# mbari-org/ecoz2rs

Hardware: AMD Instinct MI355X
Metric: vq_learn_frames_per_sec_M1024_P36 (higher is better)
Workload: dtype f64

## Files before the change

### ecoz2rs_amd/csrc/vq_pass.cpp

```cpp
#include "vq_session.h"


int e2vq_pass_mode(const e2vq_session* s)
{
    if (e2vq::uses_mfma(s->NC) && !e2vq::mfma_is_wide(s->NC)) {
        const long images = 8L * 16 * (2 * s->NC + 5 + 3) * 4;
        if ((long)s->M * s->RS * 8 + images + 2048 <= E2VQ_LDS_BYTES && s->M <= 128) return 1;
        if (s->M <= 4 * e2vq::mfma_hybrid_cells(s->NC)) return 5;
        return 2;
    }
    return 2;
}

int e2vq_fold_pending_timing(e2vq_session* s)
{
    if (!s->timing_pending) return 0;
    float ms = 0.f;
    HIPCHK(hipEventElapsedTime(&ms, s->ev0, s->ev1));
    s->timing_sum_ms += ms;
    s->timing_count += 1;
    if (s->timing_mid) HIPCHK(hipEventElapsedTime(&ms, s->ev0, s->ev_mid));
    s->timing_sweep_ms += ms;
    s->timing_mid = false;
    s->timing_pending = false;
// ... 300 lines not shown
{
    if (kind) *kind = s->last_prefiltered ? s->last_kind : 0;
    if (two_stage) *two_stage = s->last_two_stage ? 1 : 0;
    if (flagged_fraction) *flagged_fraction = s->last_flagged_frac;
    return 0;
}

extern "C" int e2vq_sweep_executed(e2vq_session* s, int64_t* flagged, int64_t* jobs, int64_t* one_stage_jobs, int reset)
{
    HIPCHK(hipSetDevice(s->device));
    u64 dev[2] = {0, 0};
    if (s->d_sort) {
        HIPCHK(hipMemcpyAsync(dev, e2vq::sweep_totals_of(s->d_sort), sizeof dev, hipMemcpyDeviceToHost, s->stream));
        if (reset) HIPCHK(hipMemsetAsync(e2vq::sweep_totals_of(s->d_sort), 0, sizeof dev, s->stream));
        HIPCHK(hipStreamSynchronize(s->stream));
    }
    if (flagged) *flagged = (int64_t)(dev[0] + s->sw_host_flagged);
    if (jobs) *jobs = (int64_t)(dev[1] + s->sw_host_jobs);
    if (one_stage_jobs) *one_stage_jobs = (int64_t)s->sw_one_stage_jobs;
    if (reset) s->sw_host_flagged = s->sw_host_jobs = s->sw_one_stage_jobs = 0;
    return 0;
}

extern "C" int e2vq_set_sweep_policy(e2vq_session* s, double two_stage_max_fraction, double max_uncertified_fraction)
{
    if (two_stage_max_fraction >= 0.0) s->two_stage_max_frac = two_stage_max_fraction;
    if (max_uncertified_fraction >= 0.0) s->pre_max_uncertified = max_uncertified_fraction;
    s->two_stage_off_until_M = 0;
    s->pre_off_from_M = 0;
    return 0;
}

extern "C" int e2vq_sweep_policy_state(e2vq_session* s, int* one_stage_until_M, int* plain_from_M, int64_t* uncertified)
{
    if (one_stage_until_M) *one_stage_until_M = s->two_stage_off_until_M;
    if (plain_from_M) *plain_from_M = s->pre_off_from_M;
    if (uncertified) *uncertified = s->last_fb;
    return 0;
}

extern "C" int e2vq_last_pass_info(e2vq_session* s, int* prefiltered, int64_t* fallback_frames)
{
    HIPCHK(hipSetDevice(s->device));
    if (prefiltered) *prefiltered = s->last_prefiltered ? 1 : 0;
    if (fallback_frames) {
        int n = 0;
// ... 222 lines not shown
        s->lstats_dirty = true;
        e2vq::launch_codebook_prepare(s->d_refl_spec, s->M, s->NC, s->d_cbq_spec, s->d_l1max_spec, s->d_cbm_spec,
                                      s->stream);
    }
    HIPCHK(hipGetLastError());
    s->spec_valid = true;
    if (spin_for_sequence(s, &s->h_stats->seq, "statistics kernel", &s->stats_wait_s)) return 1;
    if (s->rec_pending) {
        s->rec_last_total = s->h_stats->rec_total;
        s->rec_pending = false;
    }
    if (fused) {
        s->last_fb = s->last_prefiltered ? (i64)s->h_stats->fb : -1;
        const double limit = s->last_first_of_level ? std::min(1.0, 1.5 * s->pre_max_uncertified) : s->pre_max_uncertified;
        if (s->last_fb >= 0 && s->T > 0 && (double)s->last_fb > limit * (double)s->T &&
            (!s->pre_off_from_M || s->M < s->pre_off_from_M))
            s->pre_off_from_M = s->M;
    }
    if (s->sw_pending) {
        const u64 fl = s->h_stats->sw_flagged, jobs = s->h_stats->sw_jobs;
        s->sw_pending = false;
        s->sw_host_flagged += fl;
        s->sw_host_jobs += jobs;
        s->last_flagged_frac = jobs ? (double)fl / (double)jobs : -1.0;
        if (jobs && s->last_flagged_frac > s->two_stage_max_frac) s->two_stage_off_until_M = s->M;
        if (jobs && s->last_flagged_frac > 0.8 && s->last_flagged_frac > s->two_stage_max_frac)
            s->two_stage_off_until_M = (s->last_flagged_frac > 0.98 ? 4 : 2) * s->M;
    }
    i64 l[8] = {0, 0, 0, 0, 0, 0, 0, 0};
    for (int slot = 0; slot < 64; ++slot)
        for (int k = 0; k < 8; ++k) l[k] += s->h_stats->l[slot * 8 + k];
    double l1max;
    memcpy(&l1max, &s->h_stats->l1bits, 8);
    const int Ed = e2vq::dist_exponent(s->h_sc.maxabs, l1max);
    const double DD = e2vq::unfix(l[0], l[1], 30 - Ed);
    const double SS = e2vq::unfix(l[2], l[3], 30 - 2 * Ed);
    const double T = (double)s->T_total;
    const double avg = DD / T;
    const double q = SS / T;
    const double p = avg * avg;
    double v = q - p;
    if (!(v > 0.0)) v = 0.0;
    double w = 0.0;
    for (int m = 0; m < s->M; ++m) w += s->h_within[m];
    s->last.M = s->M;
    s->last.DD = DD;
// ... 62 lines not shown
```

### ecoz2rs_amd/csrc/vq_session.h

```cpp
#pragma once
#include "../../include/ecoz2_vq.h"
#include "hip_host.h"
#include "vq_device.h"
#include "vq_fixed.h"
#include "vq_io.h"
#include <hip/hip_runtime.h>
#include <dlfcn.h>
#include <errno.h>
#include <float.h>
#include <math.h>
#include <stdarg.h>
#include <stdint.h>
#include <stdio.h>
#include <stdlib.h>
#include <string.h>
#include <algorithm>
#include <chrono>
#include <atomic>
#include <condition_variable>
#include <memory>
#include <mutex>
#include <shared_mutex>
#include <string>
#include <thread>
// ... 6 lines not shown

struct e2vq_session {
    int device = 0, P = 0, NC = 0, FB = 64, RS = 0, NPAD = 0;
    hipStream_t own_stream = nullptr, stream = nullptr;
    double* d_blk = nullptr;
    double* d_aos = nullptr;
    i64 T = 0, nblocks = 0, T_total = 0;
    bool prepared = false;
    bool maxabs_scanned = false;
    int M = 0, M_cap = 0;
    double* d_refl = nullptr;
    double* d_refl_next = nullptr;
    double* d_cbq = nullptr;
    double* d_cbm = nullptr;
    double* d_cbT = nullptr;
    u64* d_l1max = nullptr;
    double* d_refl_spec = nullptr;
    double* d_cbq_spec = nullptr;
    double* d_cbm_spec = nullptr;
    u64* d_l1max_spec = nullptr;
    bool spec_valid = false;
    bool spec_zeroed = false;
    hipEvent_t ev_stats = nullptr;
    struct HostStats { i64 l[64 * 8]; u64 l1bits; volatile u64 seq; i64 failed; volatile u64 seq2; volatile u64 err; volatile i64 rec_total; volatile u64 sw_flagged, sw_jobs; volatile i64 fb; }* h_stats = nullptr;
    long verified_passes = 0;
    bool verify_publish = false;
    bool failed_pending = false;
    e2vq_level_stats* failed_patch = nullptr;
    u64 stats_seq = 0;
    double stats_wait_s = 0.0;
    double* h_within = nullptr;
    DevScalars* d_sc = nullptr;
    DevScalars h_sc{};
    u64* d_maxabs = nullptr;
    int* d_flags = nullptr;
    i64* d_stats = nullptr;
    i64* d_rows = nullptr;
    double* d_S = nullptr;
    double* d_within = nullptr;
    i64* d_lstats = nullptr;
    bool lstats_dirty = false;
    bool stats_valid = false;
    bool rows_fresh = false;
    e2vq_level_stats last{};
    double DDprv = DBL_MAX / 1e5;
    double* d_qaos = nullptr;
    double* d_qblk = nullptr;
// ... 41 lines not shown
    bool rec_enabled = true;
    int rec_min_M = 64;
    size_t rec_max_bytes = (size_t)8192 << 20;
    int rec_few_div = 3;
    bool last_recorded = false;
    bool rec_pending = false;
    bool rec_level_burst = false;
    i64 rec_last_total = -1;
    void* d_recs = nullptr;
    size_t recs_cap = 0;
    int* d_rec_counts = nullptr;
    bool sweep2_enabled = true;
    bool two_blocks_always = false;
    bool fused_enabled = true;
    int sweep_min_M = 256;
    double two_stage_max_frac = 0.45;
    double pre_max_uncertified = 0.40;
    bool last_first_of_level = false;
    int pre_off_from_M = 0;
    i64 last_fb = -1;
    int two_stage_off_until_M = 0;
    bool sw_pending = false;
    u64 sw_host_flagged = 0, sw_host_jobs = 0;
    u64 sw_one_stage_jobs = 0;
    void* d_fimgF = nullptr;
    unsigned* d_perm = nullptr;
    unsigned* d_cand = nullptr;
    void* d_sort = nullptr;
    int perm_M = 0;
    double last_flagged_frac = -1.0;
    int last_kind = 0;
    bool last_two_stage = false;
    i64* d_rows_local = nullptr;
    int rows_local_cap = 0;
    bool fam_enabled = true, fam_pending = false;
    int fam_M = 0, fam_cap = 0;
    int cells_M = 0;
    bool rows_local_is_current = false;
    bool rows_are_local = false;
    i64* d_rows_parent = nullptr;
    i64* d_fam = nullptr;
    struct Saved {
        bool valid = false;
        int M = 0, cells_M = 0, incr_M = 0;
        double DDprv = 0.0;
        bool rows_fresh = false, rows_are_local = false, rows_local_is_current = false, incr_valid = false;
// ... 33 lines not shown
```

### ecoz2rs_amd/csrc/vq_sweep.hip

```cpp
#include "vq_pre_common.h"

namespace e2vq {

template <int NC>
struct SweepImg {
    typedef PrePack<NC> PK;
    static constexpr int FS = PK::PAIRS * 32 + 32;
    static constexpr int NSTEP_C = PK::level_steps(0) + PK::level_steps(1);
    __host__ __device__ static constexpr bool coarse_unique(int u)
    {
        for (int s = 0; s < NSTEP_C; ++s)
            if (PK::step_unique(s) == u) return true;
        return false;
    }
    __host__ __device__ static constexpr bool coarse_pair(int p)
    {
        for (int s = 0; s < NSTEP_C; ++s)
            if (PK::step_pair(s) == p) return true;
        return false;
    }
    __host__ __device__ static constexpr int count_coarse_pairs()
    {
        int n = 0;
        for (int p = 0; p < PK::PAIRS; ++p) n += coarse_pair(p) ? 1 : 0;
// ... 218 lines not shown
__device__ unsigned long long g_sweep_stamps[16];
__device__ int g_sweep_exp;
#define SW_EXP(bit) ((sw_exp & (bit)) != 0)
#define SW_STAMP_DECL unsigned long long sw_acc[8] = {0, 0, 0, 0, 0, 0, 0, 0}, sw_conv = 0, sw_t = __builtin_amdgcn_s_memtime(), sw_n = 0, sw_in = 0, sw_out = 0, sw_polls = 0; \
    const int sw_exp = __builtin_amdgcn_readfirstlane(g_sweep_exp);
#define SW_STAMP(i)                                                                          \
    {                                                                                        \
        if (E2VQ_SWEEP_STAMP == 1) asm volatile("s_waitcnt vmcnt(0) lgkmcnt(0)" ::: "memory"); \
        const unsigned long long sw_now = __builtin_amdgcn_s_memtime();                     \
        sw_acc[i] += sw_now - sw_t;                                                          \
        sw_t = sw_now;                                                                       \
    }
#else
#define SW_STAMP_DECL
#define SW_STAMP(i)
#define SW_EXP(bit) false
#endif

#ifndef E2VQ_SWEEP_TOKEN_POLLS
#define E2VQ_SWEEP_TOKEN_POLLS 256
#endif
constexpr int SWEEP_TOKEN_BYTES = 16;

struct SweepCounters {
    unsigned long long flagged;
    unsigned long long jobs;
};

struct SweepFuse {
    const double* aos;
    const double* cbq;
    const DevScalars* sc;
    const u64* l1max_bits;
    unsigned short* sym;
    double* dmin;
    i64* rows;
    i64* fam;
    int* fb_list;
    unsigned short* cells;
    int incr;
    int M;
};

template <int NC>
struct SweepLds {
    static constexpr int RP0 = (NC * 8 + 15) / 16;
    static constexpr int RP = (RP0 & 1) ? RP0 : RP0 + 1;
    static constexpr int ROW_BYTES = RP * 16;
    static constexpr int ROWS_BYTES = 64 * ROW_BYTES;
    static constexpr int WAVE_BYTES_FUSE = ROWS_BYTES + 512;
// ... 23 lines not shown
    typedef const __attribute__((address_space(1))) void* gptr_t;
    typedef __attribute__((address_space(3))) void* lptr_t;
    const unsigned lds_rows = (unsigned)(unsigned long long)(lptr_t)wlds;
    int sh_r = 0, sh_d = 0, sh_d2 = 0;
    bool fast_fix = true, fast_d = true;
    double scale_r = 1.0, scale_d = 1.0, scale_d2 = 1.0;
    i64 dacc0 = 0, dacc1 = 0, dacc2 = 0, dacc3 = 0;
    if constexpr (FUSE) {
        sh_r = fz.sc->sh_r;
        const int Ed = dist_exponent(fz.sc->maxabs, __longlong_as_double((i64)*fz.l1max_bits));
        sh_d = 30 - Ed;
        sh_d2 = 30 - 2 * Ed;
        auto pow2 = [](int e) { return __longlong_as_double((long long)(1023 + e) << 52); };
        fast_fix = sh_r >= -1000 && sh_r <= 1000;
        fast_d = sh_d >= -1000 && sh_d <= 1000 && sh_d2 >= -1000 && sh_d2 <= 1000;
        scale_r = pow2(fast_fix ? sh_r : 0);
        scale_d = pow2(fast_d ? sh_d : 0);
        scale_d2 = pow2(fast_d ? sh_d2 : 0);
    }
    const float ymax1 = __int_as_float(ps->ymax_bits);
    const float relk = __int_as_float((127 + __builtin_popcount(~idxmask) - 21) << 23);
    const float pinf = __builtin_inff();
    const int col = lane & 31, h = lane >> 5;
    unsigned long long nflag = 0, njobs = 0;
    SW_STAMP_DECL
    constexpr bool TOKEN = TWO && FUSE && WAVES == 8;
    const unsigned tok_me = 1u << wib;
    unsigned* tok_w = nullptr;
    if constexpr (TOKEN) {
        unsigned* const tok = (unsigned*)(smem + (size_t)WAVES * WAVE_LDS);
        if (lane < 4) __hip_atomic_fetch_and(&tok[lane], ~tok_me, __ATOMIC_RELAXED, __HIP_MEMORY_SCOPE_WORKGROUP);
        tok_w = tok + (__builtin_amdgcn_s_getreg((2 - 1) << 11 | 4 << 6 | 4) & 3u);
    }
    auto tok_others = [&]() {
        const unsigned w = __hip_atomic_load(tok_w, __ATOMIC_RELAXED, __HIP_MEMORY_SCOPE_WORKGROUP);
        return (__builtin_amdgcn_readfirstlane((int)w) & 0xff & ~(int)tok_me) != 0;
    };
    auto tok_set = [&](bool on) {
        unsigned me = tok_me;
        asm volatile("" : "+s"(me));
        if (lane == 0) {
            if (on)
                __hip_atomic_fetch_or(tok_w, me, __ATOMIC_RELAXED, __HIP_MEMORY_SCOPE_WORKGROUP);
            else
                __hip_atomic_fetch_and(tok_w, ~me, __ATOMIC_RELAXED, __HIP_MEMORY_SCOPE_WORKGROUP);
        }
    };
// ... 40 lines not shown
#pragma unroll
        for (int hh = 0; hh < NB; ++hh) slot_frames(turn * NB + hh, fn[2 * hh], fn[2 * hh + 1]);
    };
    auto request_B = [&]() {
#pragma unroll
        for (int cb = 0; cb < NCB; ++cb) load_pairs(B[cb], g[cb], fn[cb], NB == 2 ? 5 : 7);
    };
    const long turn0 = SW_EXP(128) && wib >= 4 ? nturns : wave;
    if (turn0 < nturns) {
        next_frames(wave);
        home_n = home_of(fn[0]);
        request_B();
    }
    for (long turn = turn0; turn < nturns; turn += nwaves) {
        unsigned f[NCB];
        float gc[NCB];
#pragma unroll
        for (int cb = 0; cb < NCB; ++cb) f[cb] = fn[cb], gc[cb] = g[cb];
        const int home = home_n;
        const long tn = turn + nwaves < nturns ? turn + nwaves : turn;
        SW_STAMP(0)
        if constexpr (!TWO) next_frames(tn);
        unsigned short oldraw = 0;
        auto request_rows = [&](unsigned fs) {
            asm volatile("s_waitcnt lgkmcnt(0)" ::: "memory");
            if (fz.incr) oldraw = fz.cells[fs];
            const int lane_q = pre_fresh_lane();
            unsigned fr_next = (unsigned)__shfl((int)fs, (int)((unsigned)lane_q / (unsigned)SL::RP), 64);
#pragma unroll 1
            for (int k = 0; k < (SW_EXP(4) ? 0 : SL::RP); ++k) {
                const unsigned q = (unsigned)(k * 64 + lane_q);
                const unsigned slot = q / (unsigned)SL::RP, pc = q - slot * (unsigned)SL::RP;
                unsigned fr_ = fr_next;
                {
                    const unsigned qn = (unsigned)((k + 1 < SL::RP ? k + 1 : k) * 64 + lane_q);
                    fr_next = (unsigned)__shfl((int)fs, (int)(qn / (unsigned)SL::RP), 64);
                }
                if (SW_EXP(64)) fr_ = fs;
                if (SW_EXP(32)) fr_ &= ~1u;
                const char* gp = (const char*)fz.aos + ((size_t)fr_ * (size_t)(NC * 8) + (size_t)((pc < (unsigned)SL::RP0 ? pc : 0u) * 16u));
                __builtin_amdgcn_global_load_lds((gptr_t)gp, (lptr_t)(wlds + k * 1024), 16, 0, 0);
            }
#ifdef E2VQ_SWEEP_STAMP
            {
                const unsigned long long sw_now = __builtin_amdgcn_s_memtime();
                sw_acc[4] += sw_now - sw_t;
                sw_t = sw_now;
            }
#endif
        };
        if constexpr (FUSE) request_rows(h ? f[1] : f[0]);
        float k1[NCB], k2[NCB], k3[NCB];
        int ntl = 0;

        if constexpr (TWO) {
            auto tile_at = [&](int i) {
                i = i < MT ? i : MT - 1;
                return home + i < MT ? home + i : home + i - MT;
            };
            constexpr int ND = 2;
            if constexpr (TOKEN) {
                __builtin_amdgcn_s_setprio(0);
#pragma unroll 1
                for (int p = 0; p < E2VQ_SWEEP_TOKEN_POLLS && tok_others(); ++p) {
                    __builtin_amdgcn_s_sleep(4);
#ifdef E2VQ_SWEEP_STAMP
                    sw_polls += 1;
#endif
                }
#ifdef E2VQ_SWEEP_STAMP
                sw_in += tok_others() ? 1 : 0;
                {
                    const unsigned long long sw_now = __builtin_amdgcn_s_memtime();
                    sw_acc[0] += sw_now - sw_t;
                    sw_t = sw_now;
                }
#endif
                tok_set(true);
            }
            h8 A[ND][NU];
#pragma unroll
            for (int k = 0; k < ND - 1; ++k) sweep_load_tile<NC>(A[k], cimg, tile_at(k), lane, true);
            float U[NCB];
#pragma unroll
            for (int cb = 0; cb < NCB; ++cb) U[cb] = pinf;
            f16v acc0[2], acc1[2];
#pragma unroll
            for (int r = 0; r < 16; ++r) acc1[0][r] = 0.f, acc1[1][r] = pinf;
            unsigned bits_acc = 0u;
            int tile_prev = 0;
            auto digest = [&](float m, float& Uc, float gcb, int cb, int tile, bool valid) {
                const float Dc = 2.54f * (257.f * (gcb + ymax1) + (129.f * NC + 2.f));
                const float thrc = Uc > 0.f && Uc < pinf ? __builtin_fmaf(Uc, 1.000001f, Dc) : pinf;
                const bool fl = !(m > thrc);
                Uc = __builtin_fminf(Uc, m);
                bits_acc |= (valid && __ballot(fl) != 0) ? 1u << cb : 0u;
                if (cb == NCB - 1) {
                    if (bits_acc) {
                        tlist[ntl] = (unsigned short)((unsigned)tile | bits_acc << 8);
                        ++ntl;
                    }
                    bits_acc = 0u;
                }
            };
            for (int i0 = 0; i0 < MT; i0 += ND) {
// ... 5 lines not shown
                        const int tile = tile_at(i);
#pragma unroll
                        for (int cb = 0; cb < NCB; ++cb) {
                            const float m = (cb & 1) ? sweep_coarse_job_pinned<NC>(acc1, A[k], B[cb], acc0)
                                                     : sweep_coarse_job_pinned<NC>(acc0, A[k], B[cb], acc1);
                            if (cb == 0)
                                digest(m, U[NCB - 1], gc[NCB - 1], NCB - 1, tile_prev, i > 0);
                            else
                                digest(m, U[cb - 1], gc[cb - 1], cb - 1, tile, true);
                        }
                        tile_prev = tile;
                    }
                }
            }
            {
                float v[16];
#pragma unroll
                for (int r = 0; r < 16; ++r) v[r] = __builtin_fmaf(acc1[0][r], 512.f, acc1[1][r]);
                float m = __builtin_fminf(v[0], v[1]);
#pragma unroll
                for (int r = 2; r < 16; r += 2) m = __builtin_fminf(m, __builtin_fminf(v[r], v[r + 1]));
                digest(m, U[NCB - 1], gc[NCB - 1], NCB - 1, tile_prev, true);
            }
            njobs += (unsigned long long)NCB * MT;
            if (SW_EXP(2)) {
                ntl = 1;
                tlist[0] = (unsigned short)((unsigned)home | ((1u << NCB) - 1u) << 8);
            }
            SW_STAMP(1)
            if constexpr (TOKEN) {
                __builtin_amdgcn_s_setprio(1);
#ifdef E2VQ_SWEEP_STAMP
                sw_out += tok_others() ? 1 : 0;
#endif
                tok_set(false);
            }
            next_frames(tn);
        }
#pragma unroll
        for (int cb = 0; cb < NCB; ++cb) k1[cb] = k2[cb] = k3[cb] = __int_as_float(0x7f7fffff);
        int maskv = idxmask;
        asm volatile("" : "+v"(maskv));
        float ninf = -__builtin_inff();
        asm volatile("" : "+v"(ninf));
        if constexpr (!TWO) {
            h8 Acur[NU], Anext[NU];
            sweep_load_tile<NC>(Acur, cimg, 0, lane, false);
            for (int t = 0; t < MT; ++t) {
                sweep_load_tile<NC>(Anext, cimg, t + 1 < MT ? t + 1 : t, lane, false);
                sweep_full_job<NC>(Acur, B[0], t, k1[0], k2[0], k3[0], maskv, ninf);
                sweep_full_job<NC>(Acur, B[1], t, k1[1], k2[1], k3[1], maskv, ninf);
#pragma unroll
                for (int u = 0; u < NU; ++u) Acur[u] = Anext[u];
            }
            njobs += 2ull * MT;
            nflag += 2ull * MT;
            home_n = 0;
        }
#pragma unroll
        for (int hh = 0; hh < NB; ++hh) {
        const long b = turn * NB + hh;
        if (FUSE && hh) request_rows(h ? f[NCB - 1] : f[NCB - 2]);
        if constexpr (TWO) {
            if constexpr (NB == 2) {
                load_pairs(B[2 * hh], g[2 * hh], f[2 * hh], hh == 0 ? 2 : 3);
                load_pairs(B[2 * hh + 1], g[2 * hh + 1], f[2 * hh + 1], hh == 0 ? 2 : 3);
            }
            const unsigned sh = 8u + 2u * hh;
            auto next_e = [&](int j) {
                while (j < ntl && ((tlist[j] >> sh) & 3u) == 0u) ++j;
                return j;
            };
            int j = next_e(0);
            if (j < ntl) {
                h8 Acur[NU], Anext[NU];
                unsigned e = tlist[j];
                sweep_load_tile<NC>(Acur, cimg, (int)(e & 0xffu), lane, false);
                while (j < ntl) {
                    const int jn = next_e(j + 1);
                    const unsigned en = tlist[jn < ntl ? jn : j];
                    sweep_load_tile<NC>(Anext, cimg, (int)(en & 0xffu), lane, false);
                    const int tile = (int)(e & 0xffu);
                    const unsigned eb = e >> sh;
                    if (eb & 1u) sweep_full_job<NC>(Acur, B[2 * hh], tile, k1[2 * hh], k2[2 * hh], k3[2 * hh], maskv, ninf);
                    if (eb & 2u) sweep_full_job<NC>(Acur, B[2 * hh + 1], tile, k1[2 * hh + 1], k2[2 * hh + 1], k3[2 * hh + 1], maskv, ninf);
                    nflag += (eb & 1u) + ((eb >> 1) & 1u);
#pragma unroll
                    for (int u = 0; u < NU; ++u) Acur[u] = Anext[u];
                    e = en;
                    j = jn;
                }
            }
            if (hh == 0) home_n = home_of(fn[0]);
        }
        SW_STAMP(2)
        if constexpr (!FUSE) request_B();

        const unsigned f0 = NB == 2 && hh ? f[NCB - 2] : f[0], f1 = NB == 2 && hh ? f[NCB - 1] : f[1];
        const float gc0 = NB == 2 && hh ? gc[NCB - 2] : gc[0], gc1 = NB == 2 && hh ? gc[NCB - 1] : gc[1];
        const float ka1 = NB == 2 && hh ? k1[NCB - 2] : k1[0], ka2 = NB == 2 && hh ? k2[NCB - 2] : k2[0],
                    ka3 = NB == 2 && hh ? k3[NCB - 2] : k3[0];
// ... 26 lines not shown
        const unsigned c1 = (unsigned)(__float_as_int(t1) & ~idxmask), c2 = (unsigned)(__float_as_int(u2) & ~idxmask);
        const bool live = b * 64 + lane < T;
        if constexpr (!FUSE) {
            if (live) cand[fr] = c1 | c2 << 13 | (amb ? CAND_AMB : 0u) | (cert ? CAND_CERT : 0u);
        } else {
            double2 x[NH], y[NH];
            const unsigned la = lds_rows + (unsigned)(lane * SL::ROW_BYTES);
            {
                const double2* r1 = (const double2*)(fz.cbq + (size_t)c1 * NPAD);
                const double2* r2 = (const double2*)(fz.cbq + (size_t)c2 * NPAD);
#pragma unroll
                for (int n2 = 0; n2 < NH; ++n2) x[n2] = SW_EXP(16) ? make_double2(1.0, 1.0) : r1[n2];
#pragma unroll
                for (int n2 = 0; n2 < NH; ++n2) y[n2] = make_double2(0.0, 0.0);
                if (amb && !SW_EXP(16)) {
#pragma unroll
                    for (int n2 = 0; n2 < NH; ++n2) y[n2] = r2[n2];
                }
            }
            __builtin_amdgcn_s_waitcnt(0x0F70);
            __builtin_amdgcn_fence(__ATOMIC_ACQUIRE, "wavefront");
            asm volatile("" ::: "memory");
            double d1 = 0.0, d2 = 0.0;
#pragma unroll
            for (int b0 = 0; b0 < NC; b0 += 8) {
                double fv[8] = {0.0, 0.0, 0.0, 0.0, 0.0, 0.0, 0.0, 0.0};
#pragma unroll
                for (int k = 0; k < 8; ++k)
                    if (b0 + k < NC) asm volatile("ds_read_b64 %0, %1" : "=v"(fv[k]) : "v"(la + (unsigned)((b0 + k) * 8)));
                asm volatile("s_waitcnt lgkmcnt(0)"
                             : "+v"(fv[0]), "+v"(fv[1]), "+v"(fv[2]), "+v"(fv[3]), "+v"(fv[4]), "+v"(fv[5]), "+v"(fv[6]), "+v"(fv[7]));
#pragma unroll
                for (int k = 0; k < 8; ++k)
                    if (b0 + k < NC) {
                        d1 = __builtin_fma(fv[k], ((b0 + k) & 1) ? x[(b0 + k) >> 1].y : x[(b0 + k) >> 1].x, d1);
                        d2 = __builtin_fma(fv[k], ((b0 + k) & 1) ? y[(b0 + k) >> 1].y : y[(b0 + k) >> 1].x, d2);
                    }
                asm volatile("" : "+v"(d1), "+v"(d2));
            }
            const bool take_b = amb && (d2 < d1 || (d2 == d1 && c2 < c1));
            const double best = take_b ? d2 : d1;
            int idx = take_b ? (int)c2 : (int)c1;
            if (hh == NB - 1) request_B();
            const bool skip = !cert;
            idx = skip ? 0 : idx;
#ifdef E2VQ_SWEEP_STAMP
            {
                const unsigned long long sw_now = __builtin_amdgcn_s_memtime();
                sw_acc[5] += sw_now - sw_t;
                sw_t = sw_now;
            }
#endif
            if (live) {
                if (skip) {
                    fz.fb_list[atomicAdd(&ps->fb_count, 1)] = (int)fr;
                } else {
                    if (fz.sym) fz.sym[fr] = (unsigned short)idx;
                    if (fz.dmin) fz.dmin[fr] = best;
                    if (fz.incr != 1 || (int)oldraw != idx) fz.cells[fr] = (unsigned short)idx;
                    const double e = best - 1.0;
                    int h0, l0, h1, l1;
                    if (fast_d) {
// ... 4 lines not shown
                        fix2(e * e, sh_d2, h1, l1);
                    }
                    dacc0 += h0;
                    dacc1 += l0;
                    dacc2 += h1;
                    dacc3 += l1;
                }
            }
#ifdef E2VQ_SWEEP_STAMP
            {
                const unsigned long long sw_now = __builtin_amdgcn_s_memtime();
                sw_acc[6] += sw_now - sw_t;
                sw_t = sw_now;
            }
#endif
            {
                const int incr = fz.incr;
                const int oldc = (incr == 2 ? 2 : 1) * (int)oldraw;
                const bool mov = live && !skip && (!incr || oldc != idx);
                const bool infam = incr == 2 && idx == oldc + 1;
                const int keyN = infam ? fz.M + (oldc >> 1) : idx;
                const bool hasN = mov, hasO = mov && incr != 0 && !infam;
                u64 mN = __ballot(hasN), mO = __ballot(hasO);
                if (mov) {
                    double* fr = (double*)(wlds + lane * SL::ROW_BYTES);
                    if (fast_fix) {
#pragma unroll 4
                        for (int n = 0; n < NC; ++n) {
                            int hh, ll;
                            fix2_mul(fr[n], scale_r, hh, ll);
                            *(int2*)&fr[n] = make_int2(hh, ll);
                        }
                    } else {
#pragma unroll 1
                        for (int n = 0; n < NC; ++n) {
                            int hh, ll;
                            fix2(fr[n], sh_r, hh, ll);
                            *(int2*)&fr[n] = make_int2(hh, ll);
                        }
                    }
                }
                __builtin_amdgcn_fence(__ATOMIC_RELEASE, "wavefront");
                __builtin_amdgcn_wave_barrier();
                __builtin_amdgcn_fence(__ATOMIC_ACQUIRE, "wavefront");
#ifdef E2VQ_SWEEP_STAMP
                {
                    asm volatile("s_waitcnt lgkmcnt(0)" ::: "memory");
// ... 26 lines not shown
                    if (2 * NC > 64 && lane < 2 * NC - 64 && a1 != 0) atomicAdd((u64*)&dst[64 + lane], (u64)a1);
                    if (lane == 63 && !SW_EXP(8)) {
                        const i64 cnt = (i64)__builtin_popcountll(sN) - (i64)__builtin_popcountll(sO);
                        if (cnt != 0) atomicAdd((u64*)&dst[2 * NC], (u64)cnt);
                    }
                    mN &= ~sN;
                    mO &= ~sO;
#ifdef E2VQ_SWEEP_STAMP
                    sw_acc[7] += 1;
#endif
                }
            }
        }
#ifdef E2VQ_SWEEP_STAMP
        {
            const unsigned long long sw_now = __builtin_amdgcn_s_memtime();
            sw_acc[3] += sw_now - sw_t;
            sw_t = sw_now;
            sw_n += 1;
        }
#endif
    }
    }
#ifdef E2VQ_SWEEP_STAMP
    if (lane == 0) {
        for (int k = 0; k < 8; ++k) atomicAdd(&g_sweep_stamps[k], sw_acc[k]);
        atomicAdd(&g_sweep_stamps[8], sw_n);
        atomicAdd(&g_sweep_stamps[9], 1ull);
        atomicAdd(&g_sweep_stamps[10], nflag);
        atomicAdd(&g_sweep_stamps[11], njobs);
        atomicAdd(&g_sweep_stamps[12], sw_conv);
        atomicAdd(&g_sweep_stamps[13], sw_in);
        atomicAdd(&g_sweep_stamps[14], sw_out);
        atomicAdd(&g_sweep_stamps[15], sw_polls);
    }
#endif
    if (counters && lane == 0 && njobs) {
        atomicAdd(&counters->flagged, nflag);
        atomicAdd(&counters->jobs, njobs);
    }
    if constexpr (FUSE) {
        i64 v[4] = {dacc0, dacc1, dacc2, dacc3};
#pragma unroll
        for (int k = 0; k < 4; ++k) {
            for (int dd = 32; dd >= 1; dd >>= 1) v[k] += __shfl_xor(v[k], dd, 64);
            if (lane == 0 && v[k] != 0) atomicAdd((u64*)&fz.rows[(long)(wave % (32 * MT)) * RS + 2 * NC + 1 + k], (u64)v[k]);
        }
    }
}

template <int NC>
struct FinLds {
    static constexpr int HALF_BYTES = 32 * NC * 8;
    static constexpr int K16 = HALF_BYTES / 1024, K4 = (HALF_BYTES - K16 * 1024) / 256;
    static_assert(K16 * 1024 + K4 * 256 == HALF_BYTES, "a half block of frames is a whole number of 256-byte pieces");
    static constexpr int WAVE_BYTES = HALF_BYTES + 256;
    static constexpr int WAVES = 12;
    static_assert(WAVES * WAVE_BYTES + 512 <= E2VQ_LDS_BYTES || !PreLds<NC>::OK, "twelve half-block regions fit");
};

template <int NC>
__global__ __launch_bounds__(FinLds<NC>::WAVES * 64) void k_finish(const double* __restrict__ aos, long T, long nblocks,
                                                   const unsigned* __restrict__ cand, PreScalars* __restrict__ ps,
                                                   const double* __restrict__ cbq, int MT, const DevScalars* __restrict__ sc,
                                                   const u64* __restrict__ l1max_bits, unsigned short* __restrict__ sym,
                                                   double* __restrict__ dmin, i64* __restrict__ rows, int* __restrict__ fb_list,
                                                   unsigned short* __restrict__ prev_sym, int incr, PreRec rec,
                                                   SweepCounters* __restrict__ counters, unsigned long long* host_counters)
{
    typedef FinLds<NC> FL;
    constexpr int W = FL::WAVES;
    constexpr int RS = (2 * NC + 5 + 7) & ~7, NPAD = (NC + 7) & ~7, NH = (NC + 1) / 2;
    if (counters && host_counters && blockIdx.x == 0 && threadIdx.x == 0) {
        __hip_atomic_store(host_counters, counters->flagged, __ATOMIC_RELAXED, __HIP_MEMORY_SCOPE_SYSTEM);
        __hip_atomic_store(host_counters + 1, counters->jobs, __ATOMIC_RELAXED, __HIP_MEMORY_SCOPE_SYSTEM);
        counters->flagged = 0;
        counters->jobs = 0;
    }
    extern __shared__ __attribute__((aligned(16))) unsigned char smem[];
    const int lane = threadIdx.x & 63, wib = __builtin_amdgcn_readfirstlane((int)(threadIdx.x >> 6));
    const long wave = (long)blockIdx.x * W + wib;
    const long nwaves = (long)gridDim.x * W;
    const long nhalf = (T + 31) / 32;
    (void)nblocks;
    unsigned char* wbase = smem + (size_t)wib * FL::WAVE_BYTES;
    int* const rcnt = (int*)(smem + (size_t)W * FL::WAVE_BYTES);
    if (threadIdx.x < 64) rcnt[threadIdx.x] = 0;
    __syncthreads();
    const int Ed = dist_exponent(sc->maxabs, __longlong_as_double((i64)*l1max_bits));
    const int sh_d = 30 - Ed, sh_d2 = 30 - 2 * Ed;
    auto pow2 = [](int e) { return __longlong_as_double((long long)(1023 + e) << 52); };
    const bool fast_d = sh_d >= -1000 && sh_d <= 1000 && sh_d2 >= -1000 && sh_d2 <= 1000;
    const double scale_d = pow2(fast_d ? sh_d : 0), scale_d2 = pow2(fast_d ? sh_d2 : 0);
    const int fl = lane & 31;
    const bool second = lane >= 32;
    typedef const __attribute__((address_space(1))) void* gptr_t;
    typedef __attribute__((address_space(3))) void* lptr_t;
    const unsigned lds_rows = (unsigned)(unsigned long long)(lptr_t)wbase;
// ... 182 lines not shown
        default: return 0;
    }
}

void launch_sweep_frames(const double* aos, long T, long nblocks64, int NC, const int* ea, void* img, hipStream_t s)
{
    const long nframes = nblocks64 * 64;
    const int grid = (int)((2 * nframes + 127) / 128 < 8192 ? (2 * nframes + 127) / 128 : 8192);
    switch (NC) {
#define X(N)                                                                                                           \
    case N:                                                                                                            \
        hipLaunchKernelGGL((k_frames_fm<N>), dim3(grid), dim3(128), 0, s, aos, T, nframes, ea, (unsigned char*)img);   \
        break;
        E2VQ_PRE_NC_LIST(X)
#undef X
        default: break;
    }
}

__global__ void k_sweep_counters_out(SweepCounters* counters, unsigned long long* host)
{
    __hip_atomic_store(host, counters->flagged, __ATOMIC_RELAXED, __HIP_MEMORY_SCOPE_SYSTEM);
    __hip_atomic_store(host + 1, counters->jobs, __ATOMIC_RELAXED, __HIP_MEMORY_SCOPE_SYSTEM);
    counters->flagged = 0;
    counters->jobs = 0;
}
void launch_sweep_counters_out(void* counters, void* host_counters, hipStream_t s)
{
    hipLaunchKernelGGL(k_sweep_counters_out, dim3(1), dim3(1), 0, s, (SweepCounters*)counters, (unsigned long long*)host_counters);
}

size_t sort_scratch_bytes() { return (size_t)2 * SORT_MAX_BINS * sizeof(int) + 2 * sizeof(SweepCounters); }

int launch_sort_by_cell(const unsigned short* key, long T, long nblocks64, int nbins, void* scratch, unsigned* perm, hipStream_t s)
{
    if (nbins < 1 || nbins > SORT_MAX_BINS || T < 1) return 1;
    int* hist = (int*)scratch;
    int* cursor = hist + SORT_MAX_BINS;
    long nwg = (T + 8191) / 8192;
    nwg = nwg > 256 ? 256 : nwg;
    const long chunk = ((T + nwg - 1) / nwg + 63) / 64 * 64;
    const long used = (T + chunk - 1) / chunk;
    hipLaunchKernelGGL(k_sort_hist, dim3((unsigned)used), dim3(SORT_TPB), (size_t)nbins * sizeof(int), s, key, T, chunk, nbins, hist);
    hipLaunchKernelGGL(k_sort_base, dim3(1), dim3(SORT_TPB), 0, s, hist, nbins, cursor);
    hipLaunchKernelGGL(k_sort_scatter, dim3((unsigned)used), dim3(SORT_TPB), (size_t)2 * nbins * sizeof(int), s, key, T, chunk,
                       nbins, cursor, perm, nblocks64 * 64);
    return 0;
}
// ... 139 lines not shown
```

### ecoz2rs_amd/vq.py

```python
import ctypes as C
from dataclasses import dataclass

import numpy as np

from ._lib import ALLREDUCE_FN, LEARN_CALLBACK, LevelStatsC, c_char_pp, check, lib


def version():
    return lib.ecoz2_version().decode()


def _to_vec_of_ptr_const_c_char(paths):
    arr = (C.c_char_p * len(paths))(*[str(p).encode() for p in paths])
    return C.cast(arr, c_char_pp), arr


def _observer(callback):
    def step(_target, m, avg_distortion, sigma, inertia):
        print(f"   Ecoz2ObserverRef.step: M={m} avg_distortion={avg_distortion} sigma={sigma} inertia={inertia}")
        if callback is not None:
            callback(m, avg_distortion, sigma, inertia)

    return LEARN_CALLBACK(step)

# ... 238 lines not shown
        check(lib.e2vq_timing_total(self._h, C.byref(ms), C.byref(n)))
        return ms.value, n.value

    def timing_sweep_total(self):
        ms, n = C.c_double(), C.c_int64()
        check(lib.e2vq_timing_sweep_total(self._h, C.byref(ms), C.byref(n)))
        return ms.value, n.value

    def last_pass_records(self):
        r, n = C.c_int(), C.c_int64()
        check(lib.e2vq_last_pass_records(self._h, C.byref(r), C.byref(n)))
        return bool(r.value), n.value

    def last_pass_sweep(self):
        k, t, f = C.c_int(), C.c_int(), C.c_double()
        check(lib.e2vq_last_pass_sweep(self._h, C.byref(k), C.byref(t), C.byref(f)))
        return k.value, bool(t.value), f.value

    def sweep_executed(self, reset=False):
        f, j, o = C.c_int64(), C.c_int64(), C.c_int64()
        check(lib.e2vq_sweep_executed(self._h, C.byref(f), C.byref(j), C.byref(o), int(reset)))
        return f.value, j.value, o.value

    def set_sweep_policy(self, two_stage_max_fraction=-1.0, max_uncertified_fraction=-1.0):
        check(lib.e2vq_set_sweep_policy(self._h, float(two_stage_max_fraction), float(max_uncertified_fraction)))

    def sweep_policy_state(self):
        a, b, u = C.c_int(), C.c_int(), C.c_int64()
        check(lib.e2vq_sweep_policy_state(self._h, C.byref(a), C.byref(b), C.byref(u)))
        return a.value, b.value, u.value

    def last_pass_info(self):
        used, n = C.c_int(), C.c_int64()
        check(lib.e2vq_last_pass_info(self._h, C.byref(used), C.byref(n)))
        return bool(used.value), n.value

    def set_prev_distortion(self, dd):
        check(lib.e2vq_set_prev_distortion(self._h, float(dd)))

    def save_state(self):
        check(lib.e2vq_save_state(self._h))

    def restore_state(self):
        check(lib.e2vq_restore_state(self._h))

    def prev_distortion(self):
# ... 94 lines not shown
```

### include/ecoz2_vq.h

```cpp
#ifndef ECOZ2_VQ_H
#define ECOZ2_VQ_H

#include <stdint.h>

#ifdef __cplusplus
extern "C" {
#endif


const char *ecoz2_version(void);

typedef void (*ecoz2_vq_learn_callback_t)(void *target, int M, double avg_distortion,
                                          double sigma, double inertia);

int ecoz2_vq_learn(int prediction_order, double epsilon, const char *codebook_class_name,
                   const char *const *predictor_filenames, int num_predictors, void *target,
                   ecoz2_vq_learn_callback_t callback);

int ecoz2_vq_learn_using_base_codebook(const char *base_codebook, double epsilon,
                                       const char *const *predictor_filenames,
                                       int num_predictors, void *target,
                                       ecoz2_vq_learn_callback_t callback);

int ecoz2_vq_quantize(const char *nom_raas, const char *const *predictor_filenames,
// ... 46 lines not shown
int e2vq_group_uses_rccl(e2vq_group *g);
void e2vq_group_fail(e2vq_group *g);
void e2vq_group_destroy(e2vq_group *g);

int e2vq_set_frames_host(e2vq_session *s, const double *frames, int64_t T);
int e2vq_set_frames_device(e2vq_session *s, const void *device_frames, int64_t T);
int e2vq_prepare(e2vq_session *s);

int e2vq_set_codebook(e2vq_session *s, const double *reflections, int M);
int e2vq_get_codebook(e2vq_session *s, double *reflections, int *M);
int e2vq_init_codebook(e2vq_session *s);
int e2vq_grow(e2vq_session *s);

int e2vq_pass(e2vq_session *s, void *device_sym, void *device_dmin);
int e2vq_pass_stats(e2vq_session *s, e2vq_level_stats *out);
int e2vq_enable_timing(e2vq_session *s, int on);
int e2vq_last_pass_kernel_ms(e2vq_session *s, float *ms);
int e2vq_timing_total(e2vq_session *s, double *total_ms, int64_t *passes);
int e2vq_timing_sweep_total(e2vq_session *s, double *total_ms, int64_t *passes);
int e2vq_last_pass_info(e2vq_session *s, int *prefiltered, int64_t *fallback_frames);
int e2vq_last_pass_records(e2vq_session *s, int *recorded, int64_t *records);
int e2vq_last_pass_sweep(e2vq_session *s, int *kind, int *two_stage, double *flagged_fraction);
int e2vq_sweep_executed(e2vq_session *s, int64_t *flagged, int64_t *jobs, int64_t *one_stage_jobs, int reset);
int e2vq_set_sweep_policy(e2vq_session *s, double two_stage_max_fraction, double max_uncertified_fraction);
int e2vq_sweep_policy_state(e2vq_session *s, int *one_stage_until_M, int *plain_from_M, int64_t *uncertified);
int e2vq_sweep_launch_counts(e2vq_session *s, int64_t *prefiltered, int64_t *plain);
int e2vq_launch_counts_by_kernel(e2vq_session *s, int64_t *pass_pre_lds, int64_t *sweep_cand, int64_t *plain);
int e2vq_update(e2vq_session *s);
int e2vq_verified_passes(e2vq_session *s, int64_t *passes);
int e2vq_iterate(e2vq_session *s, void *device_sym, void *device_dmin, e2vq_level_stats *out);
int e2vq_row_stride(int prediction_order);
int e2vq_get_rows(e2vq_session *s, int64_t *rows);

int e2vq_learn(e2vq_session *s, double epsilon, int max_M, const char *class_name,
               const char *out_root, void *target, ecoz2_vq_learn_callback_t callback,
               e2vq_level_stats *levels, int max_levels, int *num_levels);

int e2vq_set_prev_distortion(e2vq_session *s, double DDprv);
int e2vq_save_state(e2vq_session *s);
int e2vq_restore_state(e2vq_session *s);
int e2vq_get_prev_distortion(e2vq_session *s, double *DDprv);

int e2vq_quantize_host(e2vq_session *s, const double *frames, int64_t T, uint16_t *sym,
                       double *dmin);
int e2vq_quantize_device(e2vq_session *s, const void *device_frames, int64_t T, void *device_sym,
                         void *device_dmin);
// ... 49 lines not shown
```

Measured before the change: 3.125 billion.

## Convert few moved frames cooperatively across lanes and reuse home tile in sweep

When fewer than a threshold of lanes in a wave have moved frames, the fixed-point row conversion is done cooperatively: all lanes walk the mover bitmask and each converts one coefficient per row, instead of each moving lane serially converting its own row. Only waves with many movers keep the per-lane path. The diff also issues the first coarse tile load before the token wait, reuses that preloaded home tile in the refinement pass, defers the cell read until after next_frames, and uses fixed LDS immediate offsets in the distance evaluation. New conversion-path counters are added and exposed to the host, which adds some atomic and bookkeeping overhead.

```diff
diff --git a/ecoz2rs_amd/csrc/vq_pass.cpp b/ecoz2rs_amd/csrc/vq_pass.cpp
--- a/ecoz2rs_amd/csrc/vq_pass.cpp
+++ b/ecoz2rs_amd/csrc/vq_pass.cpp
@@ -346,6 +346,22 @@
     return 0;
 }
 
+extern "C" int e2vq_sweep_conversion_paths(e2vq_session* s, int64_t* by_lane, int64_t* by_mover, int reset)
+{
+    HIPCHK(hipSetDevice(s->device));
+    u64 dev[2] = {0, 0};
+    if (s->d_sort) {
+        char* const words = (char*)e2vq::sweep_totals_of(s->d_sort) + 2 * sizeof(u64);
+        HIPCHK(hipMemcpyAsync(dev, words, sizeof dev, hipMemcpyDeviceToHost, s->stream));
+        if (reset) HIPCHK(hipMemsetAsync(words, 0, sizeof dev, s->stream));
+        HIPCHK(hipStreamSynchronize(s->stream));
+    }
+    if (by_lane) *by_lane = (int64_t)(dev[0] + s->sw_host_conv_lane);
+    if (by_mover) *by_mover = (int64_t)(dev[1] + s->sw_host_conv_mover);
+    if (reset) s->sw_host_conv_lane = s->sw_host_conv_mover = 0;
+    return 0;
+}
+
 extern "C" int e2vq_set_sweep_policy(e2vq_session* s, double two_stage_max_fraction, double max_uncertified_fraction)
 {
     if (two_stage_max_fraction >= 0.0) s->two_stage_max_frac = two_stage_max_fraction;
@@ -614,6 +630,8 @@
         s->sw_pending = false;
         s->sw_host_flagged += fl;
         s->sw_host_jobs += jobs;
+        s->sw_host_conv_lane += s->h_stats->sw_conv_lane;
+        s->sw_host_conv_mover += s->h_stats->sw_conv_mover;
         s->last_flagged_frac = jobs ? (double)fl / (double)jobs : -1.0;
         if (jobs && s->last_flagged_frac > s->two_stage_max_frac) s->two_stage_off_until_M = s->M;
         if (jobs && s->last_flagged_frac > 0.8 && s->last_flagged_frac > s->two_stage_max_frac)
diff --git a/ecoz2rs_amd/csrc/vq_session.h b/ecoz2rs_amd/csrc/vq_session.h
--- a/ecoz2rs_amd/csrc/vq_session.h
+++ b/ecoz2rs_amd/csrc/vq_session.h
@@ -52,7 +52,7 @@
     bool spec_valid = false;
     bool spec_zeroed = false;
     hipEvent_t ev_stats = nullptr;
-    struct HostStats { i64 l[64 * 8]; u64 l1bits; volatile u64 seq; i64 failed; volatile u64 seq2; volatile u64 err; volatile i64 rec_total; volatile u64 sw_flagged, sw_jobs; volatile i64 fb; }* h_stats = nullptr;
+    struct HostStats { i64 l[64 * 8]; u64 l1bits; volatile u64 seq; i64 failed; volatile u64 seq2; volatile u64 err; volatile i64 rec_total; volatile u64 sw_flagged, sw_jobs, sw_conv_lane, sw_conv_mover; volatile i64 fb; }* h_stats = nullptr;
     long verified_passes = 0;
     bool verify_publish = false;
     bool failed_pending = false;
@@ -140,6 +140,7 @@
     int two_stage_off_until_M = 0;
     bool sw_pending = false;
     u64 sw_host_flagged = 0, sw_host_jobs = 0;
+    u64 sw_host_conv_lane = 0, sw_host_conv_mover = 0;
     u64 sw_one_stage_jobs = 0;
     void* d_fimgF = nullptr;
     unsigned* d_perm = nullptr;
diff --git a/ecoz2rs_amd/csrc/vq_sweep.hip b/ecoz2rs_amd/csrc/vq_sweep.hip
--- a/ecoz2rs_amd/csrc/vq_sweep.hip
+++ b/ecoz2rs_amd/csrc/vq_sweep.hip
@@ -264,10 +264,46 @@
 #endif
 constexpr int SWEEP_TOKEN_BYTES = 16;
 
+template <int OFF>
+__device__ __forceinline__ void sweep_lds_read64(double& v, unsigned la)
+{
+    asm volatile("ds_read_b64 %0, %1 offset:%2" : "=v"(v) : "v"(la), "n"(OFF));
+}
+template <int NC, int B0>
+__device__ __forceinline__ void sweep_eval_batch(unsigned la, const double2 (&x)[(NC + 1) / 2], const double2 (&y)[(NC + 1) / 2], double& d1,
+                                                 double& d2)
+{
+    if constexpr (B0 < NC) {
+        double fv[8] = {0.0, 0.0, 0.0, 0.0, 0.0, 0.0, 0.0, 0.0};
+        if constexpr (B0 + 0 < NC) sweep_lds_read64<(B0 + 0) * 8>(fv[0], la);
+        if constexpr (B0 + 1 < NC) sweep_lds_read64<(B0 + 1) * 8>(fv[1], la);
+        if constexpr (B0 + 2 < NC) sweep_lds_read64<(B0 + 2) * 8>(fv[2], la);
+        if constexpr (B0 + 3 < NC) sweep_lds_read64<(B0 + 3) * 8>(fv[3], la);
+        if constexpr (B0 + 4 < NC) sweep_lds_read64<(B0 + 4) * 8>(fv[4], la);
+        if constexpr (B0 + 5 < NC) sweep_lds_read64<(B0 + 5) * 8>(fv[5], la);
+        if constexpr (B0 + 6 < NC) sweep_lds_read64<(B0 + 6) * 8>(fv[6], la);
+        if constexpr (B0 + 7 < NC) sweep_lds_read64<(B0 + 7) * 8>(fv[7], la);
+        asm volatile("s_waitcnt lgkmcnt(0)"
+                     : "+v"(fv[0]), "+v"(fv[1]), "+v"(fv[2]), "+v"(fv[3]), "+v"(fv[4]), "+v"(fv[5]), "+v"(fv[6]), "+v"(fv[7]));
+#pragma unroll
+        for (int k = 0; k < 8; ++k)
+            if (B0 + k < NC) {
+                d1 = __builtin_fma(fv[k], ((B0 + k) & 1) ? x[(B0 + k) >> 1].y : x[(B0 + k) >> 1].x, d1);
+                d2 = __builtin_fma(fv[k], ((B0 + k) & 1) ? y[(B0 + k) >> 1].y : y[(B0 + k) >> 1].x, d2);
+            }
+        asm volatile("" : "+v"(d1), "+v"(d2));
+    }
+}
+
 struct SweepCounters {
     unsigned long long flagged;
     unsigned long long jobs;
+    unsigned long long conv_lane;
+    unsigned long long conv_mover;
 };
+
+constexpr int CONV_MOVERS = 24;
+constexpr int CONV_UN = 4;
 
 struct SweepFuse {
     const double* aos;
@@ -337,7 +373,8 @@
     const float relk = __int_as_float((127 + __builtin_popcount(~idxmask) - 21) << 23);
     const float pinf = __builtin_inff();
     const int col = lane & 31, h = lane >> 5;
-    unsigned long long nflag = 0, njobs = 0;
+    unsigned long long nflag = 0;
+    int nconv_lane = 0, nconv_mover = 0;
     SW_STAMP_DECL
     constexpr bool TOKEN = TWO && FUSE && WAVES == 8;
     const unsigned tok_me = 1u << wib;
@@ -424,9 +461,9 @@
         SW_STAMP(0)
         if constexpr (!TWO) next_frames(tn);
         unsigned short oldraw = 0;
-        auto request_rows = [&](unsigned fs) {
+        auto request_rows = [&](unsigned fs, bool with_cell) {
             asm volatile("s_waitcnt lgkmcnt(0)" ::: "memory");
-            if (fz.incr) oldraw = fz.cells[fs];
+            if (with_cell && fz.incr) oldraw = fz.cells[fs];
             const int lane_q = pre_fresh_lane();
             unsigned fr_next = (unsigned)__shfl((int)fs, (int)((unsigned)lane_q / (unsigned)SL::RP), 64);
 #pragma unroll 1
@@ -451,16 +488,19 @@
             }
 #endif
         };
-        if constexpr (FUSE) request_rows(h ? f[1] : f[0]);
+        if constexpr (FUSE) request_rows(h ? f[1] : f[0], !TWO);
         float k1[NCB], k2[NCB], k3[NCB];
         int ntl = 0;
+        constexpr int ND = 2;
+        h8 A[ND][NU];
 
         if constexpr (TWO) {
             auto tile_at = [&](int i) {
-                i = i < MT ? i : MT - 1;
+                i = i < MT ? i : 0;
                 return home + i < MT ? home + i : home + i - MT;
             };
-            constexpr int ND = 2;
+#pragma unroll
+            for (int k = 0; k < ND - 1; ++k) sweep_load_tile<NC>(A[k], cimg, tile_at(k), lane, true);
             if constexpr (TOKEN) {
                 __builtin_amdgcn_s_setprio(0);
 #pragma unroll 1
@@ -480,9 +520,6 @@
 #endif
                 tok_set(true);
             }
-            h8 A[ND][NU];
-#pragma unroll
-            for (int k = 0; k < ND - 1; ++k) sweep_load_tile<NC>(A[k], cimg, tile_at(k), lane, true);
             float U[NCB];
 #pragma unroll
             for (int cb = 0; cb < NCB; ++cb) U[cb] = pinf;
@@ -534,7 +571,6 @@
                 for (int r = 2; r < 16; r += 2) m = __builtin_fminf(m, __builtin_fminf(v[r], v[r + 1]));
                 digest(m, U[NCB - 1], gc[NCB - 1], NCB - 1, tile_prev, true);
             }
-            njobs += (unsigned long long)NCB * MT;
             if (SW_EXP(2)) {
                 ntl = 1;
                 tlist[0] = (unsigned short)((unsigned)home | ((1u << NCB) - 1u) << 8);
@@ -548,6 +584,9 @@
                 tok_set(false);
             }
             next_frames(tn);
+            if constexpr (FUSE) {
+                if (fz.incr) oldraw = fz.cells[h ? f[1] : f[0]];
+            }
         }
 #pragma unroll
         for (int cb = 0; cb < NCB; ++cb) k1[cb] = k2[cb] = k3[cb] = __int_as_float(0x7f7fffff);
@@ -565,14 +604,13 @@
 #pragma unroll
                 for (int u = 0; u < NU; ++u) Acur[u] = Anext[u];
             }
-            njobs += 2ull * MT;
             nflag += 2ull * MT;
             home_n = 0;
         }
 #pragma unroll
         for (int hh = 0; hh < NB; ++hh) {
         const long b = turn * NB + hh;
-        if (FUSE && hh) request_rows(h ? f[NCB - 1] : f[NCB - 2]);
+        if (FUSE && hh) request_rows(h ? f[NCB - 1] : f[NCB - 2], true);
         if constexpr (TWO) {
             if constexpr (NB == 2) {
                 load_pairs(B[2 * hh], g[2 * hh], f[2 * hh], hh == 0 ? 2 : 3);
@@ -585,10 +623,17 @@
             };
             int j = next_e(0);
             if (j < ntl) {
-                h8 Acur[NU], Anext[NU];
+                h8 Acur[NU];
                 unsigned e = tlist[j];
-                sweep_load_tile<NC>(Acur, cimg, (int)(e & 0xffu), lane, false);
+                if (hh == 0 && (int)(e & 0xffu) == home) {
+                    const h8* src = cimg + (size_t)home * PK::TILE_E + lane;
+#pragma unroll
+                    for (int u = 0; u < NU; ++u) Acur[u] = SweepImg<NC>::coarse_unique(u) ? A[0][u] : src[u * 64];
+                } else {
+                    sweep_load_tile<NC>(Acur, cimg, (int)(e & 0xffu), lane, false);
+                }
                 while (j < ntl) {
+                    h8 Anext[NU];
                     const int jn = next_e(j + 1);
                     const unsigned en = tlist[jn < ntl ? jn : j];
                     sweep_load_tile<NC>(Anext, cimg, (int)(en & 0xffu), lane, false);
@@ -661,22 +706,15 @@
             __builtin_amdgcn_fence(__ATOMIC_ACQUIRE, "wavefront");
             asm volatile("" ::: "memory");
             double d1 = 0.0, d2 = 0.0;
-#pragma unroll
-            for (int b0 = 0; b0 < NC; b0 += 8) {
-                double fv[8] = {0.0, 0.0, 0.0, 0.0, 0.0, 0.0, 0.0, 0.0};
-#pragma unroll
-                for (int k = 0; k < 8; ++k)
-                    if (b0 + k < NC) asm volatile("ds_read_b64 %0, %1" : "=v"(fv[k]) : "v"(la + (unsigned)((b0 + k) * 8)));
-                asm volatile("s_waitcnt lgkmcnt(0)"
-                             : "+v"(fv[0]), "+v"(fv[1]), "+v"(fv[2]), "+v"(fv[3]), "+v"(fv[4]), "+v"(fv[5]), "+v"(fv[6]), "+v"(fv[7]));
-#pragma unroll
-                for (int k = 0; k < 8; ++k)
-                    if (b0 + k < NC) {
-                        d1 = __builtin_fma(fv[k], ((b0 + k) & 1) ? x[(b0 + k) >> 1].y : x[(b0 + k) >> 1].x, d1);
-                        d2 = __builtin_fma(fv[k], ((b0 + k) & 1) ? y[(b0 + k) >> 1].y : y[(b0 + k) >> 1].x, d2);
-                    }
-                asm volatile("" : "+v"(d1), "+v"(d2));
-            }
+            sweep_eval_batch<NC, 0>(la, x, y, d1, d2);
+            sweep_eval_batch<NC, 8>(la, x, y, d1, d2);
+            sweep_eval_batch<NC, 16>(la, x, y, d1, d2);
+            sweep_eval_batch<NC, 24>(la, x, y, d1, d2);
+            sweep_eval_batch<NC, 32>(la, x, y, d1, d2);
+            sweep_eval_batch<NC, 40>(la, x, y, d1, d2);
+            sweep_eval_batch<NC, 48>(la, x, y, d1, d2);
+            sweep_eval_batch<NC, 56>(la, x, y, d1, d2);
+            static_assert(NC <= 64, "eight batches of eight coefficients");
             const bool take_b = amb && (d2 < d1 || (d2 == d1 && c2 < c1));
             const double best = take_b ? d2 : d1;
             int idx = take_b ? (int)c2 : (int)c1;
@@ -727,7 +765,47 @@
                 const int keyN = infam ? fz.M + (oldc >> 1) : idx;
                 const bool hasN = mov, hasO = mov && incr != 0 && !infam;
                 u64 mN = __ballot(hasN), mO = __ballot(hasO);
-                if (mov) {
+                const int nmov = (int)__builtin_popcountll(mN);
+                if (nmov != 0 && nmov < CONV_MOVERS) {
+                    nconv_mover = __builtin_amdgcn_readfirstlane(nconv_mover + 1);
+                    u64 w = mN;
+                    int ln = lane;
+                    asm volatile("" : "+v"(ln));
+                    if (fast_fix) {
+#pragma unroll 1
+                        for (int it = 0; it < 64 / CONV_UN && w != 0; ++it) {
+                            int ro[CONV_UN];
+                            double xv[CONV_UN];
+#pragma unroll
+                            for (int k = 0; k < CONV_UN; ++k) {
+                                ro[k] = w != 0 ? (int)__builtin_ctzll(w) * SL::ROW_BYTES : -1;
+                                w &= w - 1;
+                            }
+#pragma unroll
+                            for (int k = 0; k < CONV_UN; ++k) xv[k] = ro[k] >= 0 && ln < NC ? *(const double*)(wlds + ro[k] + ln * 8) : 0.0;
+#pragma unroll
+                            for (int k = 0; k < CONV_UN; ++k) {
+                                int hh, ll;
+                                fix2_mul(xv[k], scale_r, hh, ll);
+                                if (ro[k] >= 0 && ln < NC) *(int2*)(wlds + ro[k] + ln * 8) = make_int2(hh, ll);
+                            }
+                        }
+                    } else {
+#pragma unroll 1
+                        for (int it = 0; it < 64 && w != 0; ++it) {
+                            double* const row = (double*)(wlds + (int)__builtin_ctzll(w) * SL::ROW_BYTES);
+                            w &= w - 1;
+                            if (ln < NC) {
+                                int hh, ll;
+                                fix2(row[ln], sh_r, hh, ll);
+                                *(int2*)&row[ln] = make_int2(hh, ll);
+                            }
+                        }
+                    }
+                } else if (nmov != 0) {
+                    nconv_lane = __builtin_amdgcn_readfirstlane(nconv_lane + 1);
+                }
+                if (mov && nmov >= CONV_MOVERS) {
                     double* fr = (double*)(wlds + lane * SL::ROW_BYTES);
                     if (fast_fix) {
 #pragma unroll 4
@@ -800,6 +878,8 @@
 #endif
     }
     }
+    const unsigned long long njobs =
+        turn0 < nturns ? (unsigned long long)((nturns - turn0 + nwaves - 1) / nwaves) * (unsigned long long)(NCB * MT) : 0ull;
 #ifdef E2VQ_SWEEP_STAMP
     if (lane == 0) {
         for (int k = 0; k < 8; ++k) atomicAdd(&g_sweep_stamps[k], sw_acc[k]);
@@ -816,6 +896,8 @@
     if (counters && lane == 0 && njobs) {
         atomicAdd(&counters->flagged, nflag);
         atomicAdd(&counters->jobs, njobs);
+        if (nconv_lane) atomicAdd(&counters->conv_lane, (unsigned long long)nconv_lane);
+        if (nconv_mover) atomicAdd(&counters->conv_mover, (unsigned long long)nconv_mover);
     }
     if constexpr (FUSE) {
         i64 v[4] = {dacc0, dacc1, dacc2, dacc3};
@@ -852,6 +934,8 @@
     if (counters && host_counters && blockIdx.x == 0 && threadIdx.x == 0) {
         __hip_atomic_store(host_counters, counters->flagged, __ATOMIC_RELAXED, __HIP_MEMORY_SCOPE_SYSTEM);
         __hip_atomic_store(host_counters + 1, counters->jobs, __ATOMIC_RELAXED, __HIP_MEMORY_SCOPE_SYSTEM);
+        __hip_atomic_store(host_counters + 2, 0ull, __ATOMIC_RELAXED, __HIP_MEMORY_SCOPE_SYSTEM);
+        __hip_atomic_store(host_counters + 3, 0ull, __ATOMIC_RELAXED, __HIP_MEMORY_SCOPE_SYSTEM);
         counters->flagged = 0;
         counters->jobs = 0;
     }
@@ -1080,8 +1164,9 @@
 {
     __hip_atomic_store(host, counters->flagged, __ATOMIC_RELAXED, __HIP_MEMORY_SCOPE_SYSTEM);
     __hip_atomic_store(host + 1, counters->jobs, __ATOMIC_RELAXED, __HIP_MEMORY_SCOPE_SYSTEM);
-    counters->flagged = 0;
-    counters->jobs = 0;
+    __hip_atomic_store(host + 2, counters->conv_lane, __ATOMIC_RELAXED, __HIP_MEMORY_SCOPE_SYSTEM);
+    __hip_atomic_store(host + 3, counters->conv_mover, __ATOMIC_RELAXED, __HIP_MEMORY_SCOPE_SYSTEM);
+    *counters = SweepCounters{};
 }
 void launch_sweep_counters_out(void* counters, void* host_counters, hipStream_t s)
 {
diff --git a/ecoz2rs_amd/vq.py b/ecoz2rs_amd/vq.py
--- a/ecoz2rs_amd/vq.py
+++ b/ecoz2rs_amd/vq.py
@@ -284,6 +284,13 @@
         check(lib.e2vq_sweep_executed(self._h, C.byref(f), C.byref(j), C.byref(o), int(reset)))
         return f.value, j.value, o.value
 
+    def sweep_conversion_paths(self, reset=False):
+        fn = lib.e2vq_sweep_conversion_paths
+        fn.restype, fn.argtypes = C.c_int, [C.c_void_p, C.POINTER(C.c_int64), C.POINTER(C.c_int64), C.c_int]
+        a, b = C.c_int64(), C.c_int64()
+        check(fn(self._h, C.byref(a), C.byref(b), int(reset)))
+        return a.value, b.value
+
     def set_sweep_policy(self, two_stage_max_fraction=-1.0, max_uncertified_fraction=-1.0):
         check(lib.e2vq_set_sweep_policy(self._h, float(two_stage_max_fraction), float(max_uncertified_fraction)))
 
diff --git a/include/ecoz2_vq.h b/include/ecoz2_vq.h
--- a/include/ecoz2_vq.h
+++ b/include/ecoz2_vq.h
@@ -92,6 +92,7 @@
 int e2vq_last_pass_records(e2vq_session *s, int *recorded, int64_t *records);
 int e2vq_last_pass_sweep(e2vq_session *s, int *kind, int *two_stage, double *flagged_fraction);
 int e2vq_sweep_executed(e2vq_session *s, int64_t *flagged, int64_t *jobs, int64_t *one_stage_jobs, int reset);
+int e2vq_sweep_conversion_paths(e2vq_session *s, int64_t *by_lane, int64_t *by_mover, int reset);
 int e2vq_set_sweep_policy(e2vq_session *s, double two_stage_max_fraction, double max_uncertified_fraction);
 int e2vq_sweep_policy_state(e2vq_session *s, int *one_stage_until_M, int *plain_from_M, int64_t *uncertified);
 int e2vq_sweep_launch_counts(e2vq_session *s, int64_t *prefiltered, int64_t *plain);
```

Result: no change. 3.149 billion (median of 6 runs) (+0.8%).
